# facebookresearch/gtn

Hardware: AMD Instinct MI355X
Metric: CTC forward+backward losses/sec (T=1000, C=256) (higher is better)
Workload: dtype f32; 1 GPU; BASELINE config C3: compose(ctc_target, emissions)+forwardScore CTC loss fwd+bwd, T=1000, C=256, U=100, batch=512 per GPU; global_batch=512, parallelism=dp1 (utterance sharding, all_gather of losses), rccl_ranks=0

## Files before the change

gtn_amd/csrc/band.hip:

```cpp
#include <hip/hip_runtime.h>

#include <algorithm>
#include <cstdlib>
#include <stdexcept>
#include <type_traits>

#include "kernels.h"

#ifdef GTNX_BAND_TIMING
__device__ long long g_band_timing[256];
#endif

namespace gtnx {
namespace {

constexpr float NEGF = -1.0e30f;
constexpr float DEADF = -1.0e29f;
constexpr float LOG2E = 1.44269504088896340736f;
constexpr double LN2 = 0.693147180559945309417;
constexpr int BW = 256;
constexpr int WG = 512;
constexpr int WGB = 768;
constexpr int NBE = 5;
constexpr int NBG = 7;
constexpr int NBGE = 8;
#ifndef GTNX_BWD_SPLIT
#define GTNX_BWD_SPLIT 0
#endif
#ifndef GTNX_FWD_COPY_DEPTH
// ... 323 lines not shown
    P.norm = nullptr;
    P.em_copy = nullptr;
    P.grad_em = pt.grad_em ? pt.grad_em + int64_t(b) * pt.A : nullptr;
    P.grad_fixed = pt.grad_fixed ? pt.grad_fixed + P.goff : nullptr;
  }
  return P;
}
template <int NPL, bool UNIT, bool GRADG, int K, bool VEC, bool BIG>
__global__ __launch_bounds__(WGB, BIG ? 3 : 6) void band_backward_kernel(const BandPair* __restrict__ pairs, int NSmax, BandPatch patch) {
#define GTNX_BAND_PAIR band_patched(pairs[blockIdx.x], patch)
#include "band_backward_body.inc"
#undef GTNX_BAND_PAIR
}
template <int NPL, bool UNIT, bool GRADG, int K, bool VEC, bool BIG>
__global__ __launch_bounds__(WGB, BIG ? 3 : 6) void band_backward_one_kernel(BandPair one, int NSmax) {
#define GTNX_BAND_PAIR one
#include "band_backward_body.inc"
#undef GTNX_BAND_PAIR
}


__global__ __launch_bounds__(512) void ctc_targets_kernel(const CtcTargetArgs* __restrict__ args, int blank) {
  const CtcTargetArgs a = args[blockIdx.x];
  __shared__ __attribute__((aligned(16))) int tl[256 + 4];
  __shared__ __attribute__((aligned(16))) int tk[256 + 4];
  const int N = a.N, U = (N - 1) >> 1, m = threadIdx.x;
  if (m < 260) {
    const int v = m < U ? a.labels[m] : 0x7fffffff;
    tl[m] = v;
    tk[m] = (m > 0 && m < U && v != a.labels[m - 1]) ? 1 : 0;
  }
  __syncthreads();
  if (m >= N) return;
  const bool odd = (m & 1) != 0;
  const int my = odd ? tl[(m - 1) >> 1] : blank;
  const int skip = odd ? tk[(m - 1) >> 1] : 0;
  const int mi = (m - 1) >> 1;
  const int before = odd ? mi : (m >> 1);
  int rank = 0, skips = 0;
  for (int o = 0; o < U; o += 4) {
    const gtnx_i4 l4 = *reinterpret_cast<const gtnx_i4*>(tl + o), k4 = *reinterpret_cast<const gtnx_i4*>(tk + o);
    const int lo[4] = {l4.x, l4.y, l4.z, l4.w}, ko[4] = {k4.x, k4.y, k4.z, k4.w};
#pragma unroll
    for (int k = 0; k < 4; ++k) {
      const bool front = o + k < before;
      rank += (lo[k] < my || (lo[k] == my && front)) ? 1 : 0;
      skips += front ? ko[k] : 0;
    }
  }
  rank += blank < my ? U + 1 : (blank == my ? (m + 1) >> 1 : 0);
  const int base = (m > 0 ? 2 * m - 1 : 0) + skips;
  GTNX_G BandNode* nd = const_cast<GTNX_G BandNode*>(a.nodes);
  nd[m].lab = my;
  nd[m].aid[0] = base;
  nd[m].aid[1] = m > 0 ? base + 1 : -1;
  nd[m].aid[2] = skip ? base + 2 : -1;
  a.nflags[m] = uint8_t((m == 0 ? NF_START : 0) | (m + 2 >= N ? NF_ACCEPT : 0));
  a.snode[rank] = m;
  a.slab[rank] = my;
  if (m == N - 1 && a.n_arcs) a.n_arcs[0] = base + 1 + (m > 0 ? 1 : 0) + skip;
}

__global__ __launch_bounds__(512) void band_viterbi_kernel(const BandDecode* __restrict__ pairs) {
  const BandDecode P = pairs[blockIdx.x];
  const int T = P.T, C = P.C, N = P.N, NS = P.NS;
  extern __shared__ float lds[];
  const float NINF = -__builtin_inff();
  float* a0 = lds;
  float* a1 = lds + 516;
  float* stage = lds + 1032;
  const int m = threadIdx.x;
  const GTNX_G gtnx_i4* nodes = reinterpret_cast<const GTNX_G gtnx_i4*>(P.nodes);
  int lab = 0;
  float wi[3] = {NINF, NINF, NINF};
  bool accept = false, start = false;
  if (m < N) {
    const gtnx_i4 q = nodes[m];
    lab = q.x >= 0 ? q.x : 0;
    const int a[3] = {q.y, q.z, q.w};
#pragma unroll
    for (int k = 0; k < 3; ++k)
      if (a[k] >= 0) wi[k] = P.w ? P.w[a[k]] : 0.0f;
    const uint8_t f = P.nflags[m];
// ... 565 lines not shown
```

gtn_amd/csrc/batch.cpp:

```cpp
#include "batch.h"

#include <algorithm>
#include <atomic>
#include <cstdlib>
#include <cstring>
#include <limits>
#include <unordered_map>
#include <unordered_set>

namespace gtnx {

namespace {

std::atomic<uint64_t> g_batch_seq{1};

struct CompMode {
  int old;
  CompMode() : old(compose_mode_hint(2)) {}
  ~CompMode() { compose_mode_hint(old); }
};

BatchP make_batch(Batch::Kind k, int n, bool cg) {
  auto b = std::make_shared<Batch>();
  b->kind = k;
  b->n = n;
  b->calc_grad = cg;
  return b;
}

BatchP result(Batch::Kind k, int n, std::shared_ptr<BatchOp> op) {
  bool cg = false;
  for (auto& i : op->inputs) cg |= i->calc_grad;
  BatchP r = make_batch(k, n, cg);
  op->seq = g_batch_seq.fetch_add(1);
  r->op = std::move(op);
  return r;
}

bool native(const Batch& b, Batch::Kind k) { return b.kind == k; }

void pad_fill(Batch& b, float* base, const int64_t* offs = nullptr) {
  if (b.kind != Batch::LINEAR || b.pad_floats <= 0) return;
  Runtime& rt = Runtime::get();
  const size_t n = size_t(b.n);
  const size_t rows_bytes = align_up(sizeof(int) * n, 256);
  if (!b.pad_mem) {
    std::vector<int64_t> tab(rows_bytes / 8 + n + 1);
    std::memcpy(tab.data(), b.rows.data(), sizeof(int) * n);
    int64_t* prefix = tab.data() + rows_bytes / 8;
    prefix[0] = 0;
    for (size_t i = 0; i < n; ++i) prefix[i + 1] = prefix[i] + int64_t(b.M - b.rows[i]) * b.C;
    b.pad_mem = upload_vec(tab);
  }
  PadFillArgs a{};
  a.base = base;
  a.rows = b.pad_mem->as<int>();
  a.prefix = reinterpret_cast<const int64_t*>(b.pad_mem->as<char>(rows_bytes));
  a.stride = int64_t(b.M) * b.C;
  a.n = b.n;
  a.C = b.C;
  DevMemP d_offs;
  if (offs) {
// ... 351 lines not shown
  b->lab_off.resize(size_t(n) + 1);
  b->lab_off[0] = 0;
  for (int i = 0; i < n; ++i) {
    if (lengths[i] < 0) throw_invalid("[gtnx_batch_ctc_targets] negative length");
    b->lab_off[size_t(i) + 1] = b->lab_off[size_t(i)] + lengths[i];
    b->max_nodes = std::max(b->max_nodes, 2 * lengths[i] + 1);
  }
  const size_t total = size_t(b->lab_off[size_t(n)]);
  b->labels.assign(labels, labels + total);
  int mn = blank;
  b->max_label = blank;
  for (size_t i = 0; i < total; ++i) {
    b->max_label = std::max(b->max_label, labels[i]);
    mn = std::min(mn, labels[i]);
  }
  if (mn < 0 || b->max_nodes > band_max_nodes() || n == 0) {
    std::vector<Graph> gs;
    gs.reserve(size_t(n));
    for (int i = 0; i < n; ++i)
      gs.push_back(ctc_target_graph_host(labels + b->lab_off[size_t(i)], lengths[i], blank, calc_grad));
    return batch_from_graphs(std::move(gs));
  }
  Runtime& rt = Runtime::get();
  const size_t lab_bytes = align_up(sizeof(int) * (total ? total : 1), 256);
  const size_t arg_bytes = align_up(sizeof(CtcTargetArgs) * size_t(n), 256);
  size_t bytes = lab_bytes + arg_bytes;
  b->rec_off.resize(size_t(n));
  for (int i = 0; i < n; ++i) {
    const size_t N = size_t(2 * lengths[i] + 1);
    b->rec_off[size_t(i)] = bytes;
    bytes += align_up(sizeof(BandNode) * N, 64) + align_up(N, 64) + 2 * align_up(4 * N, 64) + 64;
  }
  b->rec_mem = rt.alloc(bytes);
  PinnedMemP pin = rt.alloc_pinned(lab_bytes + arg_bytes);
  std::memcpy(pin->ptr, labels, sizeof(int) * total);
  CtcTargetArgs* args = reinterpret_cast<CtcTargetArgs*>(static_cast<char*>(pin->ptr) + lab_bytes);
  for (int i = 0; i < n; ++i) {
    const size_t N = size_t(2 * lengths[i] + 1);
    char* base = b->rec_mem->as<char>(b->rec_off[size_t(i)]);
    CtcTargetArgs& a = args[size_t(i)];
    a.labels = b->rec_mem->as<int>() + b->lab_off[size_t(i)];
    a.nodes = reinterpret_cast<BandNode*>(base);
    base += align_up(sizeof(BandNode) * N, 64);
    a.nflags = reinterpret_cast<uint8_t*>(base);
    base += align_up(N, 64);
    a.snode = reinterpret_cast<int*>(base);
    base += align_up(4 * N, 64);
    a.slab = reinterpret_cast<int*>(base);
    base += align_up(4 * N, 64);
    a.n_arcs = reinterpret_cast<int*>(base);
    a.N = int(N);
    a.pad = 0;
  }
  rt.h2d_pinned(b->rec_mem->ptr, pin->ptr, lab_bytes + arg_bytes);
  launch_ctc_targets(reinterpret_cast<const CtcTargetArgs*>(b->rec_mem->as<char>(lab_bytes)), n, blank, rt.stream());
  return b;
}


BatchP batch_asg_force_align(const int* labels, const int* lengths, int n, Graph& transitions, int n_labels) {
  if (n < 0) throw_invalid("[gtnx_batch_asg_force_align] negative batch size");
  if (transitions.num_nodes() != int64_t(n_labels) + 1 || transitions.num_arcs() != int64_t(n_labels) * (n_labels + 1))
    throw_invalid("[gtnx_batch_asg_force_align] the transitions graph must have the asgTransitions(N) layout");
  BatchP b = make_batch(Batch::CTC_TARGETS, n, transitions.calc_grad());
  b->fal = true;
  b->trans = transitions;
  b->trans_labels = n_labels;
  b->lab_off.resize(size_t(n) + 1);
  b->lab_off[0] = 0;
  int max_u = 0;
  for (int i = 0; i < n; ++i) {
    if (lengths[i] < 0) throw_invalid("[gtnx_batch_asg_force_align] negative length");
    b->lab_off[size_t(i) + 1] = b->lab_off[size_t(i)] + lengths[i];
    max_u = std::max(max_u, lengths[i]);
  }
  b->max_nodes = max_u + 1;
  const size_t total = size_t(b->lab_off[size_t(n)]);
  b->labels.assign(labels, labels + total);
// ... 520 lines not shown
      p.T = ch.rows_of(b);
      p.C = C;
      p.NS = band_row_stride(p.N, band_npl(p.N));
      p.alpha = op->arena->as<float>(ao[size_t(b)]);
      p.aoff = op->arena->as<double>(oo[size_t(b)]);
      p.score = op->arena->as<float>(4 * size_t(b));
      if (want_norm) {
        p.norm = op->arena->as<float>(o_norm + 4 * size_t(b));
        p.rowlse = op->arena->as<float>(o_lse + 4 * size_t(b) * size_t(T));
      }
      p.hot = (!fx.fal && U + 1 >= 8) ? fx.blank : -1;
      p.lgrn = band_forward_lgrn(C);
      p.bidx = b;
      p.goff = goff_run;
      goff_run += int64_t(fx.elem_size(b));
      BandPair q = p;
      if (fuse_copy) {
        q.em = static_cast<const float*>(pend->src_of(p.em));
        q.em_copy = const_cast<float*>(p.em);
      }
      tab.push_back({BandLaunchKey{C, band_npl(q.N), fx.fal ? 0 : 1, 0, band_vec_ok(q)}, q});
      abytes += 4.0 * p.T * C + 4.0 * double(p.T + 1) * p.NS + (fuse_copy ? 4.0 * T * C : 0.0);
    }
    band_launch(tab, false, "band_forward_score", abytes, fuse_copy ? nullptr : &op->fwd_table);
    if (fuse_copy) pend->done.store(true, std::memory_order_release);
    if (want_norm) {
      ch.nc_mem = op->arena;
      ch.nc_norm = op->arena->as<float>(o_norm);
      ch.nc_rowlse = op->arena->as<float>(o_lse);
    }
    DevMemP arena = op->arena;
    BatchP r = result(Batch::SCALAR, n, op);
    r->v_mem = arena;
    r->v_dev = arena->as<float>();
    return r;
  }
  if (!tropical && native(*x, Batch::LINEAR) && !x->materialised && x->nc_norm) {
    auto op = std::make_shared<BFsLinearOp>();
    op->inputs = {x};
    BatchP r = result(Batch::SCALAR, x->n, op);
    r->v_mem = x->nc_mem;
    r->v_dev = x->nc_norm;
    return r;
  }
  if (!tropical && native(*x, Batch::LINEAR) && !x->materialised && x->n > 0 && x->M > 0) {
    if (x->w_pend) x->w_pend->settle();
    auto op = std::make_shared<BFsLinearOp>();
// ... 105 lines not shown
  bool asg = x->kind == Batch::PRODUCT && x->fixed && x->chain && x->fixed->kind == Batch::CTC_TARGETS && x->fixed->fal &&
             x->chain->kind == Batch::LINEAR && x->fixed->rec_mem && x->fixed->n == n && x->chain->n == n;
  if (asg) {
    const Batch& fx = *x->fixed;
    const Batch& ch = *x->chain;
    const int vec = ch.C % 4 == 0 && (reinterpret_cast<uintptr_t>(ch.w_dev) & 15) == 0;
    asg = asg_align_ok(fx.max_nodes, ch.C, vec) && fx.trans_labels == ch.C && fx.max_label < ch.C;
  }
  if (!fast && !asg) {
    align_fallback(x, frames, labels_dev, row_stride, tokens_dev, scores_dev);
    return;
  }
  Batch& fx = *x->fixed;
  Batch& ch = *x->chain;
  const int T = ch.M, C = ch.C;
  if (row_stride < T) throw_invalid("[gtnx_batch_viterbi_align] row_stride is shorter than the chains");
  if (frames)
    for (int b = 0; b < n; ++b) {
      if (frames[b] < 0 || frames[b] > T) throw_invalid("[gtnx_batch_viterbi_align] a frame count outside 0 .. T");
      if (frames[b] > ch.rows_of(b))
        throw_invalid("[gtnx_batch_viterbi_align] a frame count beyond the rows the chain carries");
    }
  if (ch.w_pend) ch.w_pend->settle();
  if (asg) {
    const int npl = asg_align_npl(fx.max_nodes);
    const size_t plane = asg_align_plane_bytes(T, npl);
    DevMemP work = rt.alloc(plane * size_t(n));
    std::vector<AsgAlignArgs> tab(static_cast<size_t>(n));
    double abytes = 0;
    for (int b = 0; b < n; ++b) {
      AsgAlignArgs& a = tab[size_t(b)];
      a = AsgAlignArgs{};
      const int U = fx.lab_off[size_t(b) + 1] - fx.lab_off[size_t(b)];
      const size_t N = size_t(U) + 1;
      char* base = fx.rec_mem->as<char>(fx.rec_off[size_t(b)]);
      a.nodes = reinterpret_cast<BandNode*>(base);
      a.nflags = reinterpret_cast<uint8_t*>(base + align_up(sizeof(BandNode) * N, 64));
      a.w = fx.rec_mem->as<float>(fx.w_off[size_t(b)]);
      a.em = ch.w_dev + size_t(b) * size_t(T) * size_t(C);
      a.bp = work->as<unsigned>(plane * size_t(b));
      a.labels = labels_dev + int64_t(b) * row_stride;
      a.tokens = tokens_dev ? tokens_dev + int64_t(b) * row_stride : nullptr;
      a.score = scores_dev ? scores_dev + b : nullptr;
      a.N = int(N);
      a.T = frames ? frames[b] : ch.rows_of(b);
      a.T_full = T;
// ... 604 lines not shown
  const bool binary = k != SK_NEGATE;
  if (binary && a->n == b->n) {
    const bool an = a->kind == Batch::SCALAR && !a->materialised, bn = b->kind == Batch::SCALAR && !b->materialised;
    if (an && !bn && b->kind == Batch::GRAPHS) {
      if (BatchP w = scalars_from_graphs(b)) b = w;
    } else if (bn && !an && a->kind == Batch::GRAPHS) {
      if (BatchP w = scalars_from_graphs(a)) a = w;
    }
  }

  if (native(*a, Batch::SCALAR) && !a->materialised &&
      (!binary || (native(*b, Batch::SCALAR) && !b->materialised && b->n == a->n))) {
    Runtime& rt = Runtime::get();
    auto op = std::make_shared<BScalarOp>();
    op->kind = k;
    op->inputs = binary ? std::vector<BatchP>{a, b} : std::vector<BatchP>{a};
    BatchP r = result(Batch::SCALAR, a->n, op);
    if (items_dev) {
      r->v_dev = static_cast<float*>(items_dev);
    } else {
      r->v_mem = rt.alloc(sizeof(float) * size_t(a->n ? a->n : 1));
      r->v_dev = r->v_mem->as<float>();
    }
    launch_vec_axpby(r->v_dev, a->v_dev, binary ? b->v_dev : nullptr, size_t(a->n), k == SK_NEGATE ? -1.0f : 1.0f,
                     k == SK_SUBTRACT ? -1.0f : 1.0f, 0, rt.stream());
    return r;
  }
  batch_materialise(*a);
  std::vector<Graph> none;
  if (binary) batch_materialise(*b);
  BatchP r = batch_from_graphs(op_scalar(k, a->graphs, binary ? b->graphs : none));
  if (items_dev) batch_items_device(r, items_dev);
  return r;
}

void batch_backward(const BatchP& root, bool retain) {
  GTNX_HOST_T("batch.backward");
  if (root->tape_cleared)
    throw_invalid("[autograd::backward] Cannot Backward twice without retaining the graph.");
  if (root->materialised || !root->op || root->kind != Batch::SCALAR) {
    batch_materialise(*root);
    op_backward(root->graphs, nullptr, retain);
    return;
  }
  Runtime& rt = Runtime::get();
  std::vector<Batch*> order;
  std::unordered_set<Batch*> seen;
  std::vector<BatchP> hold;
  std::vector<BatchP> stack{root};
  while (!stack.empty()) {
    BatchP b = stack.back();
    stack.pop_back();
    if (!b->calc_grad || !seen.insert(b.get()).second) continue;
    hold.push_back(b);
    if (b->op) {
      order.push_back(b.get());
      for (auto& in : b->op->inputs) stack.push_back(in);
    }
  }
  std::sort(order.begin(), order.end(), [](Batch* a, Batch* b) { return a->op->seq > b->op->seq; });
  bool root_done = false;
  if (!root->g_dev) {
    alloc_grad(*root, false);
    auto* sop = dynamic_cast<BScalarOp*>(root->op.get());
    bool plain = sop != nullptr && !sop->inputs.empty() && sop->inputs.size() <= 2;
    if (plain)
      for (auto& in : sop->inputs) plain = plain && in->kind == Batch::SCALAR && !in->materialised && in->n == root->n;
    if (plain && sop->inputs.size() == 2 && sop->inputs[0].get() == sop->inputs[1].get()) plain = false;
    if (plain) {
      float* g[2] = {nullptr, nullptr};
      float sc[2] = {0.0f, 0.0f};
      int acc[2] = {0, 0};
      for (size_t i = 0; i < sop->inputs.size(); ++i) {
        Batch& in = *sop->inputs[i];
        if (!in.calc_grad) continue;
        sc[i] = (sop->kind == SK_NEGATE || (sop->kind == SK_SUBTRACT && i == 1)) ? -1.0f : 1.0f;
        acc[i] = in.g_dev != nullptr;
        if (!in.g_dev) alloc_grad(in, false);
        g[i] = in.g_dev;
      }
      launch_scalar_seed(root->g_dev, g[0], sc[0], acc[0], g[1], sc[1], acc[1], size_t(root->n), rt.stream());
      root_done = true;
    } else {
      launch_fill_f32(root->g_dev, 1.0f, size_t(root->n), rt.stream());
    }
  } else {
    DevMemP ones = rt.alloc(sizeof(float) * size_t(root->n ? root->n : 1));
    launch_fill_f32(ones->as<float>(), 1.0f, size_t(root->n), rt.stream());
    launch_vec_axpby(root->g_dev, ones->as<float>(), nullptr, size_t(root->n), 1.0f, 0.0f, 1, rt.stream());
  }
  std::vector<Batch*> from_graphs;
  BackwardPlan plan;
  t_plan = &plan;
  struct RetainScope {
    bool prev;
    explicit RetainScope(bool r) : prev(t_batch_retain) { t_batch_retain = r; }
    ~RetainScope() { t_batch_retain = prev; }
  } retain_scope(retain);
  try {
    for (Batch* b : order) {
      if (!b->g_dev) continue;
      if (root_done && b == root.get()) continue;
      if (auto* f = dynamic_cast<BFromGraphsOp*>(b->op.get())) {
        f->retain = retain;
        from_graphs.push_back(b);
        continue;
// ... 114 lines not shown
```

gtn_amd/csrc/batch.h:

```cpp
#pragma once

#include <memory>
#include <vector>

#include "ops.h"

namespace gtnx {

struct Batch;
using BatchP = std::shared_ptr<Batch>;

struct BatchOp {
  uint64_t seq = 0;
  std::vector<BatchP> inputs;
  virtual void backward(Batch& out) = 0;
  virtual ~BatchOp() {}
};

struct Batch {
  enum Kind { GRAPHS, CTC_TARGETS, LINEAR, PRODUCT, SCALAR };
  Kind kind = GRAPHS;
  int n = 0;
  bool calc_grad = false;

  bool materialised = false;
  std::vector<Graph> graphs;
  bool leaf = false;
  struct Origin {
    std::shared_ptr<void> home;
    size_t begin, end;
  };
  std::vector<Origin> origins;
  void (*give_back)(const std::shared_ptr<void>& home, std::vector<Graph>* part) = nullptr;
  std::vector<float> host_vals;
  bool host_vals_valid = false;
  PinnedMemP host_pin;
  void* host_ev = nullptr;

  std::vector<int> labels, lab_off;
  int blank = 0;
  int max_label = -1, max_nodes = 0;
  DevMemP rec_mem;
  std::vector<size_t> rec_off;
  bool fal = false;
  Graph trans;
  int trans_labels = 0;
  std::vector<size_t> w_off, map_off;
  int M = 0, C = 0;
  DevMemP w_mem;
  float* w_dev = nullptr;
  std::shared_ptr<PendingCopy> w_pend;
  DevMemP nc_mem;
  float* nc_norm = nullptr;
  float* nc_rowlse = nullptr;
  std::vector<int> rows;
  int64_t pad_floats = 0;
  DevMemP pad_mem;
  int rows_of(int b) const { return rows.empty() ? M : rows[size_t(b)]; }
  BatchP fixed, chain;
  bool chain_first = false, intersect = false;
  bool wide = false;
  bool full = false;
  DevMemP v_mem;
  float* v_dev = nullptr;

  std::shared_ptr<BatchOp> op;
  bool tape_cleared = false;
  DevMemP g_mem;
  float* g_dev = nullptr;
  std::vector<int64_t> g_off;
  DevMemP dest_mem;
  float* dest = nullptr;

  int64_t elem_size(int b) const;
  ~Batch();
};

BatchP batch_from_graphs(std::vector<Graph> gs);
BatchP batch_ctc_targets(const int* labels, const int* lengths, int n, int blank, bool calc_grad);
BatchP batch_asg_force_align(const int* labels, const int* lengths, int n, Graph& transitions, int n_labels);
BatchP batch_linear(int n, int M, int C, bool calc_grad, const void* dev, bool borrow, const int* rows = nullptr);
BatchP batch_compose(const BatchP& a, const BatchP& b, bool intersect);
BatchP batch_shortest_distance(const BatchP& x, bool tropical);
void batch_full_connect_stats(int64_t* fast, int64_t* fallback);
BatchP batch_viterbi_path(const BatchP& x);
void batch_viterbi_align(const BatchP& x, const int* frames, int* labels_dev, int64_t row_stride, int* tokens_dev,
                         float* scores_dev);
// ... 35 lines not shown
```

gtn_amd/csrc/kernels.h:

```cpp
#pragma once

#include <hip/hip_runtime.h>

#include <cstdint>

#include <atomic>
#include <cstdint>
struct gtnx_first_on_device {
  std::atomic<uint64_t>& done;
  uint64_t bit;
  bool first;
  explicit gtnx_first_on_device(std::atomic<uint64_t>& d) : done(d) {
    int dev = 0;
    (void)hipGetDevice(&dev);
    bit = uint64_t(1) << (dev & 63);
    first = !(done.load(std::memory_order_acquire) & bit);
  }
  gtnx_first_on_device(const gtnx_first_on_device&) = delete;
  ~gtnx_first_on_device() {
    if (first) done.fetch_or(bit, std::memory_order_acq_rel);
  }
  explicit operator bool() const { return first; }
};

// ... 449 lines not shown
  GTNX_G int* stamp;
  GTNX_G int* queue;
  GTNX_G int* arc_cnt;
  const GTNX_G int* arc_off;
  RationalOut out;
};
void launch_remove_keep(const DGraph& g, int ilabel, int olabel, int* keep, hipStream_t st);
void launch_remove_roots(const int* keep, const int* new_id, int N, int* roots, hipStream_t st);
void launch_remove_walk(const RemoveArgs& a, bool emit, hipStream_t st);
size_t scan_temp_bytes(int n);
void launch_exclusive_scan(const int* in, int* out, int n, void* temp, size_t temp_bytes, hipStream_t st);
void launch_rational_load(const void* rows, const float* w, const uint8_t* flags, const RationalOut& out, void* temp,
                          hipStream_t st);
struct CtcTargetArgs {
  const GTNX_G int* labels;
  GTNX_G BandNode* nodes;
  GTNX_G uint8_t* nflags;
  GTNX_G int* snode;
  GTNX_G int* slab;
  GTNX_G int* n_arcs;
  int N, pad;
};
void launch_ctc_targets(const CtcTargetArgs* d_args, int n, int blank, hipStream_t st);
struct AsgFalArgs {
  const GTNX_G int* labels;
  const GTNX_G float* trans_w;
  GTNX_G BandNode* nodes;
  GTNX_G uint8_t* nflags;
  GTNX_G int* snode;
  GTNX_G int* slab;
  GTNX_G float* w;
  GTNX_G int* arc_map;
  int U, pad;
};
void launch_asg_fal_targets(const AsgFalArgs* d_args, int n, int n_labels, hipStream_t st);
void launch_asg_fal_scatter(const float* g, const int* maps, const int64_t* tab , int n_seq, int64_t longest,
                            float* trans_grad, hipStream_t st);
int band_max_nodes();
int band_max_labels();
int band_min_labels();
int band_npl(int max_nodes);
int band_row_stride(int N, int npl);
int band_forward_lgrn(int C);
bool band_one_ok(int npl, int C, int max_NS, bool vec, bool backward);
void launch_band_forward(const BandPair* d_pairs, int n, int npl, int C, int max_NS, bool unit, bool vec, hipStream_t st,
                         const BandPair* one = nullptr);
// ... 5 lines not shown
void launch_lazy_dense_fixed_grad(const LazyGroup& g, hipStream_t st);
size_t maxplus_w_floats(const LazyGroup& g);
void launch_maxplus_prep(const LazyGroup& g, hipStream_t st);
void launch_maxplus_step(const LazyGroup& g, int t, hipStream_t st);
void launch_maxplus_path(const LazyGroup& g, int* path_arc, int* path_il, int* path_ol, float* path_w, int* path_len,
                         hipStream_t st);
void launch_asg_decode(const LazyGroup& g, const int* d_frames, int* labels, int64_t row_stride, float* scores,
                       int* collapsed, int* lengths, hipStream_t st);
void launch_lazy_mfma_prep(const LazyGroup& g, hipStream_t st);
void launch_lazy_mfma_init(const LazyGroup& g, int which, hipStream_t st);
void launch_lazy_mfma_step(const LazyGroup& g, int t, int backward, hipStream_t st);
size_t lazy_mfma_chain_sync_ints(const LazyGroup& g);
bool launch_lazy_mfma_chain(const LazyGroup& g, int backward, int* zeroed_sync, int cus, hipStream_t st);
void launch_lazy_mfma_keys(float* keys, int64_t n, hipStream_t st);
void launch_lazy_mfma_rowmax(const LazyGroup& g, int which, hipStream_t st);
void launch_lazy_mfma_score(const LazyGroup& g, hipStream_t st);
size_t lazy_mfma_fixed_grad_scratch_bytes(const LazyGroup& g);
void launch_lazy_mfma_fixed_grad(const LazyGroup& g, void* pair_consts , hipStream_t st, void* partials = nullptr,
                                 size_t partials_bytes = 0);

void launch_fill_i32(int* p, int v, size_t n, hipStream_t st);
void launch_fill_f32(float* p, float v, size_t n, hipStream_t st);
void launch_scalar_seed(float* root, float* g0, float s0, int acc0, float* g1, float s1, int acc1, size_t n, hipStream_t st);
struct ScalarArgs {
  const GTNX_G float* a;
  const GTNX_G float* b;
  GTNX_G float* out;
  GTNX_G float* mirror;
};
void launch_scalar_combine(const ScalarArgs* d_args, int n, float sa, float sb, hipStream_t st);
void launch_copy_small(void* dst, const void* src, size_t bytes, hipStream_t st);
void launch_scalar_combine_one(const ScalarArgs& a, float sa, float sb, hipStream_t st);
struct ScalarFanArgs {
  const GTNX_G float* d;
  GTNX_G float* seed;
  GTNX_G float* o0;
  GTNX_G float* o1;
};
void launch_scalar_fan(const ScalarFanArgs* d_args, int n, float s0, float s1, hipStream_t st);
void launch_scalar_fan_one(const ScalarFanArgs& a, float s0, float s1, hipStream_t st);
struct AxpyArgs {
  GTNX_G float* dst;
  const GTNX_G float* src;
  int64_t n;
  float scale;
};
// ... 104 lines not shown
```

gtn_amd/csrc/ops.h:

```cpp
#pragma once

#include <cstring>
#include <tuple>
#include <vector>

#include "graph.h"

namespace gtnx {

struct Member {
  int idx;
  Graph out;
};

struct OpRecord {
  uint64_t seq = 0;
  virtual void backward(std::vector<Member>& members) = 0;
  virtual bool joins_chain_plan() const { return false; }
  virtual ~OpRecord() {}
};

struct GradSink {
  struct Item {
    Graph g;
    DevMemP owner;
    float* ptr;
  };
  std::vector<Item> items;
  void add(const Graph& g, const DevMemP& owner, float* ptr) {
    if (g.calc_grad()) items.push_back({g, owner, ptr});
  }
  void flush();
};

struct BandLaunchKey {
  int C, npl, unit, gradg, vec;
  bool operator<(const BandLaunchKey& o) const {
    return std::tie(C, npl, unit, gradg, vec) < std::tie(o.C, o.npl, o.unit, o.gradg, o.vec);
  }
  bool operator==(const BandLaunchKey& o) const { return !(*this < o) && !(o < *this); }
};
int band_vec_ok(const BandPair& p);
void band_launch(std::vector<std::pair<BandLaunchKey, BandPair>>& tab, bool backward, const char* prof_name = nullptr,
                 double prof_bytes = 0.0, DevMemP* table_out = nullptr);
void band_launch_patched(const DevMemP& table, int n, const BandLaunchKey& key, int max_ns, const BandPatch& patch,
                         const char* prof_name, double prof_bytes);

enum ScalarKind { SK_NEGATE = 0, SK_ADD = 1, SK_SUBTRACT = 2 };

std::vector<Graph> op_scalar(ScalarKind k, std::vector<Graph>& a, std::vector<Graph>& b);
std::vector<Graph> op_shortest_distance(std::vector<Graph>& gs, bool tropical);
std::vector<Graph> op_viterbi_path(std::vector<Graph>& gs);
std::vector<Graph> op_compose(std::vector<Graph>& a, std::vector<Graph>& b, bool intersect);
bool lazy_decode_ok(Graph& fixed, int M, int C);
void lazy_viterbi_decode(std::vector<Graph>& chains, Graph& fixed, const std::vector<int>& frames, int* labels_dev,
                         int64_t row_stride, float* scores_dev, int* collapsed_dev, int* lengths_dev);
enum RationalKind { RAT_CLONE = 0, RAT_CONCAT = 1, RAT_CLOSURE = 2, RAT_UNION = 3 };
Graph op_rational(int kind, std::vector<Graph>& inputs, int projection);
Graph op_remove(Graph& g, int ilabel, int olabel);
Graph op_load_buffer(const void* data, size_t bytes);
void op_backward(std::vector<Graph>& roots, Graph* grad, bool retain, bool seed = true);
void backward_validate(Graph& root);
int compose_mode_hint(int mode);
void realize(Graph& g);

Graph make_scalar_graph(float v, bool calc_grad);
Graph make_linear_graph(int M, int N, bool calc_grad);
// ... 41 lines not shown
```

gtn_amd/csrc/ops_band.cpp:

```cpp
#include "ops_internal.h"

#include <memory>

namespace gtnx {

int band_vec_ok(const BandPair& p) { return p.C % 4 == 0 && (reinterpret_cast<uintptr_t>(p.em) & 15) == 0; }
void band_launch_patched(const DevMemP& table, int n, const BandLaunchKey& k, int max_ns, const BandPatch& patch,
                         const char* prof_name, double prof_bytes) {
  Runtime& rt = Runtime::get();
  std::unique_ptr<Runtime::Scope> prof(prof_name ? new Runtime::Scope(&rt, prof_name, prof_bytes) : nullptr);
  launch_band_backward(table->as<BandPair>(), n, k.npl, k.C, max_ns, k.unit != 0, k.gradg != 0, k.vec != 0, rt.stream(), nullptr,
                       &patch);
}
void band_launch(std::vector<std::pair<BandLaunchKey, BandPair>>& tab, bool backward, const char* prof_name, double prof_bytes,
                 DevMemP* table_out) {
  Runtime& rt = Runtime::get();
  if (table_out) table_out->reset();
  if (tab.empty()) return;
  bool one_key = true;
  for (size_t i = 1; i < tab.size() && one_key; ++i) one_key = tab[i].first == tab[0].first;
  if (!one_key) std::stable_sort(tab.begin(), tab.end(), [](const auto& x, const auto& y) { return x.first < y.first; });
  if (tab.size() == 1) {
    const BandLaunchKey& k = tab[0].first;
    const BandPair& p = tab[0].second;
    if (band_one_ok(k.npl, k.C, p.NS, k.vec != 0, backward)) {
      std::unique_ptr<Runtime::Scope> prof(prof_name ? new Runtime::Scope(&rt, prof_name, prof_bytes) : nullptr);
      if (backward) launch_band_backward(nullptr, 1, k.npl, k.C, p.NS, k.unit != 0, k.gradg != 0, true, rt.stream(), &p);
      else launch_band_forward(nullptr, 1, k.npl, k.C, p.NS, k.unit != 0, true, rt.stream(), &p);
      return;
    }
  }
  std::vector<BandPair> flat;
  flat.reserve(tab.size());
  for (auto& e : tab) flat.push_back(e.second);
  DevMemP d = upload_vec(flat);
// ... 692 lines not shown
```

gtn_amd/csrc/runtime.cpp:

```cpp
#include "runtime.h"

#include "kernels.h"

#include <malloc.h>

#include <atomic>
#include <condition_variable>
#include <cstring>
#include <deque>
#include <thread>

namespace gtnx {

namespace {
constexpr int kMaxDevices = 64;
std::atomic<Runtime*> g_rts[kMaxDevices];
std::atomic<bool> g_any_rt{false};
std::mutex g_rt_mu;
std::atomic<int> g_default_device{-1};
thread_local int t_device = -1;

int hip_device_now() {
  int d = -1;
  if (hipGetDevice(&d) != hipSuccess) {
// ... 562 lines not shown
    (void)hipGetLastError();
    return false;
  }
  return a.type == hipMemoryTypeHost || (a.type == hipMemoryTypeDevice && a.device == dev);
}
}
bool ptr_local_to(const void* p, int dev) { return local_to(p, dev); }
void Runtime::d2d(void* dst, const void* src, size_t bytes) {
  if (!bytes) return;
  if (bytes <= (size_t(1) << 20) && local_to(src, device_) && local_to(dst, device_)) {
    launch_copy_small(dst, src, bytes, stream_);
    return;
  }
  HIP_CHECK(hipMemcpyAsync(dst, src, bytes, hipMemcpyDeviceToDevice, stream_));
}
void Runtime::d2h_pinned_async(void* pinned_dst, const void* src, size_t bytes) {
  if (!bytes) return;
  if (bytes <= (size_t(1) << 20) && local_to(src, device_)) {
    launch_copy_small(pinned_dst, src, bytes, stream_);
    return;
  }
  HIP_CHECK(hipMemcpyAsync(pinned_dst, src, bytes, hipMemcpyDeviceToHost, stream_));
}
void Runtime::h2d_pinned(void* dst, const void* pinned_src, size_t bytes) {
  if (!bytes) return;
  static const size_t lim = [] {
    const char* e = std::getenv("GTNX_H2D_KERNEL_BYTES");
    return e ? size_t(std::atol(e)) : size_t(1) << 20;
  }();
  if (bytes <= lim && local_to(dst, device_)) {
    launch_copy_small(dst, pinned_src, bytes, stream_);
    return;
  }
  HIP_CHECK(hipMemcpyAsync(dst, pinned_src, bytes, hipMemcpyHostToDevice, stream_));
}

Runtime::MirrorSlot Runtime::mirror_slot() {
  {
    std::lock_guard<std::mutex> lk(mu_);
    if (!mirror_ring_) {
      OnDevice here(device_);
      void* p = nullptr;
      HIP_CHECK(hipHostMalloc(&p, sizeof(float) * kMirrorSlots, hipHostMallocDefault));
      mirror_gen_ = new std::atomic<uint64_t>[kMirrorSlots];
      for (size_t i = 0; i < kMirrorSlots; ++i) mirror_gen_[i].store(0);
      mirror_ring_ = static_cast<float*>(p);
    }
  }
  const uint64_t g = mirror_next_.fetch_add(1) + 1;
  const size_t i = size_t(g % kMirrorSlots);
  mirror_gen_[i].store(g);
  return {mirror_ring_ + i, g};
// ... 126 lines not shown
```

gtn_amd/csrc/runtime.h:

```cpp
#pragma once

#include <atomic>
#include <functional>
#include <map>
#include <memory>
#include <mutex>
#include <string>
#include <vector>

#include "common.h"

namespace gtnx {

class Runtime;

struct DevMem {
  void* ptr = nullptr;
  size_t bytes = 0;
  bool borrowed = false;
  Runtime* owner = nullptr;
  std::shared_ptr<void> keep;
  ~DevMem();
  template <class T>
  T* as(size_t byte_off = 0) const { return reinterpret_cast<T*>(static_cast<char*>(ptr) + byte_off); }
// ... 46 lines not shown
    bool dead = false;
  };
  using InboxP = std::shared_ptr<Inbox>;
  static InboxP home();
  static void send(const InboxP& to, void* p, void (*del)(void*));
  static void drain_all_inboxes();
  static void defer_delete(void* p, void (*del)(void*), size_t weight = 1);
  static void drain_deferred();
  static bool drain_some(size_t max_items);
  static size_t deferred_count();
  void drain_until(void* hip_event);
  void drain_while_busy();
  void sync_while_draining();

  struct SideJob;
  using SideJobP = std::shared_ptr<SideJob>;
  SideJobP side_launch(std::function<void(hipStream_t)> fn);
  void side_join(const SideJobP& job);

  void h2d(void* dst, const void* src, size_t bytes);
  void d2h_sync(void* dst, const void* src, size_t bytes);
  void d2d(void* dst, const void* src, size_t bytes);
  void h2d_pinned(void* dst, const void* pinned_src, size_t bytes);
  void d2h_pinned_async(void* pinned_dst, const void* src, size_t bytes);

  struct MirrorSlot {
    float* ptr = nullptr;
    uint64_t gen = 0;
  };
  static constexpr size_t kMirrorSlots = 1024;
  MirrorSlot mirror_slot();
  bool mirror_read(const MirrorSlot& m, float* out);

  void prof_enable(bool on);
  void prof_add_bytes(const std::string& name, double bytes);
  void prof_reset();
  bool prof_on() const { return prof_on_; }
  struct Scope {
    Runtime* rt;
    int idx;
    Scope(Runtime* r, const char* name, double bytes);
    ~Scope();
  };
  ProfEntry prof_get(const std::string& name);
  std::string prof_names();
  int cu_count() const { return cu_count_; }
// ... 56 lines not shown
```

Before: 1.036 million losses/s.

## Fuse CTC target staging, pair-table upload and loss seeding into fewer launches

The CTC target builder now reads labels and args directly from pinned host staging inside a single head kernel. That kernel also copies the forward band pair table, so the separate H2D copy and table upload launches are folded into it and deferred until the forward score launch. For the subtract loss, a fused seed kernel computes the difference and writes the root and input gradient seeds at once, and backward adopts these instead of launching a fill or seed kernel. This cuts kernel launch and host overhead per step but adds state (head_pin, seed_mem) and an env switch, and the kernels now read host-pinned memory over the bus.

```diff
diff --git a/gtn_amd/csrc/band.hip b/gtn_amd/csrc/band.hip
--- a/gtn_amd/csrc/band.hip
+++ b/gtn_amd/csrc/band.hip
@@ -5,6 +5,7 @@
 #include <stdexcept>
 #include <type_traits>
 
+#include "ctc_targets_build.h"
 #include "kernels.h"
 
 #ifdef GTNX_BAND_TIMING
@@ -374,43 +375,7 @@
 
 __global__ __launch_bounds__(512) void ctc_targets_kernel(const CtcTargetArgs* __restrict__ args, int blank) {
   const CtcTargetArgs a = args[blockIdx.x];
-  __shared__ __attribute__((aligned(16))) int tl[256 + 4];
-  __shared__ __attribute__((aligned(16))) int tk[256 + 4];
-  const int N = a.N, U = (N - 1) >> 1, m = threadIdx.x;
-  if (m < 260) {
-    const int v = m < U ? a.labels[m] : 0x7fffffff;
-    tl[m] = v;
-    tk[m] = (m > 0 && m < U && v != a.labels[m - 1]) ? 1 : 0;
-  }
-  __syncthreads();
-  if (m >= N) return;
-  const bool odd = (m & 1) != 0;
-  const int my = odd ? tl[(m - 1) >> 1] : blank;
-  const int skip = odd ? tk[(m - 1) >> 1] : 0;
-  const int mi = (m - 1) >> 1;
-  const int before = odd ? mi : (m >> 1);
-  int rank = 0, skips = 0;
-  for (int o = 0; o < U; o += 4) {
-    const gtnx_i4 l4 = *reinterpret_cast<const gtnx_i4*>(tl + o), k4 = *reinterpret_cast<const gtnx_i4*>(tk + o);
-    const int lo[4] = {l4.x, l4.y, l4.z, l4.w}, ko[4] = {k4.x, k4.y, k4.z, k4.w};
-#pragma unroll
-    for (int k = 0; k < 4; ++k) {
-      const bool front = o + k < before;
-      rank += (lo[k] < my || (lo[k] == my && front)) ? 1 : 0;
-      skips += front ? ko[k] : 0;
-    }
-  }
-  rank += blank < my ? U + 1 : (blank == my ? (m + 1) >> 1 : 0);
-  const int base = (m > 0 ? 2 * m - 1 : 0) + skips;
-  GTNX_G BandNode* nd = const_cast<GTNX_G BandNode*>(a.nodes);
-  nd[m].lab = my;
-  nd[m].aid[0] = base;
-  nd[m].aid[1] = m > 0 ? base + 1 : -1;
-  nd[m].aid[2] = skip ? base + 2 : -1;
-  a.nflags[m] = uint8_t((m == 0 ? NF_START : 0) | (m + 2 >= N ? NF_ACCEPT : 0));
-  a.snode[rank] = m;
-  a.slab[rank] = my;
-  if (m == N - 1 && a.n_arcs) a.n_arcs[0] = base + 1 + (m > 0 ? 1 : 0) + skip;
+  ctc_targets_build<false>(a, a.labels, blank);
 }
 
 __global__ __launch_bounds__(512) void band_viterbi_kernel(const BandDecode* __restrict__ pairs) {
diff --git a/gtn_amd/csrc/batch.cpp b/gtn_amd/csrc/batch.cpp
--- a/gtn_amd/csrc/batch.cpp
+++ b/gtn_amd/csrc/batch.cpp
@@ -1,4 +1,5 @@
 #include "batch.h"
+#include "ctc_head.h"
 
 #include <algorithm>
 #include <atomic>
@@ -38,6 +39,36 @@
 }
 
 bool native(const Batch& b, Batch::Kind k) { return b.kind == k; }
+
+bool step_fused() {
+  static const bool on = [] {
+    const char* e = std::getenv("GTNX_STEP_LAUNCHES");
+    return !(e && std::atoi(e) == 7);
+  }();
+  return on;
+}
+
+void launch_head(Batch& fx, const BandPair* pairs, DevMemP* table) {
+  Runtime& rt = Runtime::get();
+  CtcHeadArgs h{};
+  h.stage = fx.head_pin->ptr;
+  h.dev = fx.rec_mem->ptr;
+  h.arg_off = fx.head_arg_off;
+  h.n = fx.n;
+  h.blank = fx.blank;
+  if (pairs) {
+    h.pair_bytes = ctc_head_put_pairs(fx.head_pair_off, fx.head_pin->ptr, pairs, fx.n);
+    DevMemP d = rt.alloc(h.pair_bytes);
+    h.pair_src = fx.head_pin->as<char>(fx.head_pair_off);
+    h.pair_dst = d->ptr;
+    *table = std::move(d);
+  }
+  launch_ctc_head(h, rt.stream());
+  fx.head_pin.reset();
+}
+void settle_head(Batch& fx) {
+  if (fx.head_pin) launch_head(fx, nullptr, nullptr);
+}
 
 void pad_fill(Batch& b, float* base, const int64_t* offs = nullptr) {
   if (b.kind != Batch::LINEAR || b.pad_floats <= 0) return;
@@ -435,38 +466,20 @@
     return batch_from_graphs(std::move(gs));
   }
   Runtime& rt = Runtime::get();
-  const size_t lab_bytes = align_up(sizeof(int) * (total ? total : 1), 256);
-  const size_t arg_bytes = align_up(sizeof(CtcTargetArgs) * size_t(n), 256);
-  size_t bytes = lab_bytes + arg_bytes;
-  b->rec_off.resize(size_t(n));
-  for (int i = 0; i < n; ++i) {
-    const size_t N = size_t(2 * lengths[i] + 1);
-    b->rec_off[size_t(i)] = bytes;
-    bytes += align_up(sizeof(BandNode) * N, 64) + align_up(N, 64) + 2 * align_up(4 * N, 64) + 64;
-  }
-  b->rec_mem = rt.alloc(bytes);
-  PinnedMemP pin = rt.alloc_pinned(lab_bytes + arg_bytes);
-  std::memcpy(pin->ptr, labels, sizeof(int) * total);
-  CtcTargetArgs* args = reinterpret_cast<CtcTargetArgs*>(static_cast<char*>(pin->ptr) + lab_bytes);
-  for (int i = 0; i < n; ++i) {
-    const size_t N = size_t(2 * lengths[i] + 1);
-    char* base = b->rec_mem->as<char>(b->rec_off[size_t(i)]);
-    CtcTargetArgs& a = args[size_t(i)];
-    a.labels = b->rec_mem->as<int>() + b->lab_off[size_t(i)];
-    a.nodes = reinterpret_cast<BandNode*>(base);
-    base += align_up(sizeof(BandNode) * N, 64);
-    a.nflags = reinterpret_cast<uint8_t*>(base);
-    base += align_up(N, 64);
-    a.snode = reinterpret_cast<int*>(base);
-    base += align_up(4 * N, 64);
-    a.slab = reinterpret_cast<int*>(base);
-    base += align_up(4 * N, 64);
-    a.n_arcs = reinterpret_cast<int*>(base);
-    a.N = int(N);
-    a.pad = 0;
-  }
-  rt.h2d_pinned(b->rec_mem->ptr, pin->ptr, lab_bytes + arg_bytes);
-  launch_ctc_targets(reinterpret_cast<const CtcTargetArgs*>(b->rec_mem->as<char>(lab_bytes)), n, blank, rt.stream());
+  const CtcHeadLayout lay = ctc_head_layout(lengths, n, total);
+  b->rec_off = lay.rec_off;
+  b->rec_mem = rt.alloc(lay.dev_bytes);
+  const bool head = step_fused() && n > 1 && lay.stage_bytes(true) <= Runtime::h2d_kernel_limit();
+  PinnedMemP pin = rt.alloc_pinned(lay.stage_bytes(head));
+  ctc_head_fill(lay, pin->ptr, b->rec_mem->ptr, labels, b->lab_off.data(), lengths, n);
+  if (head) {
+    b->head_pin = std::move(pin);
+    b->head_arg_off = lay.lab_bytes;
+    b->head_pair_off = lay.pair_off();
+    return b;
+  }
+  rt.h2d_pinned(b->rec_mem->ptr, pin->ptr, lay.stage_bytes(false));
+  launch_ctc_targets(reinterpret_cast<const CtcTargetArgs*>(b->rec_mem->as<char>(lay.lab_bytes)), n, blank, rt.stream());
   return b;
 }
 
@@ -1033,7 +1046,24 @@
       tab.push_back({BandLaunchKey{C, band_npl(q.N), fx.fal ? 0 : 1, 0, band_vec_ok(q)}, q});
       abytes += 4.0 * p.T * C + 4.0 * double(p.T + 1) * p.NS + (fuse_copy ? 4.0 * T * C : 0.0);
     }
-    band_launch(tab, false, "band_forward_score", abytes, fuse_copy ? nullptr : &op->fwd_table);
+    bool one_group = n > 1;
+    int max_ns = 0;
+    for (auto& e : tab) {
+      one_group = one_group && e.first == tab[0].first;
+      max_ns = std::max(max_ns, e.second.NS);
+    }
+    if (fx.head_pin && one_group) {
+      std::vector<BandPair> flat;
+      flat.reserve(tab.size());
+      for (auto& e : tab) flat.push_back(e.second);
+      DevMemP table;
+      launch_head(fx, flat.data(), &table);
+      if (!fuse_copy) op->fwd_table = table;
+      band_launch_forward_table(table, n, tab[0].first, max_ns, "band_forward_score", abytes);
+    } else {
+      settle_head(fx);
+      band_launch(tab, false, "band_forward_score", abytes, fuse_copy ? nullptr : &op->fwd_table);
+    }
     if (fuse_copy) pend->done.store(true, std::memory_order_release);
     if (want_norm) {
       ch.nc_mem = op->arena;
@@ -1185,6 +1215,7 @@
         throw_invalid("[gtnx_batch_viterbi_align] a frame count beyond the rows the chain carries");
     }
   if (ch.w_pend) ch.w_pend->settle();
+  settle_head(fx);
   if (asg) {
     const int npl = asg_align_npl(fx.max_nodes);
     const size_t plane = asg_align_plane_bytes(T, npl);
@@ -1835,6 +1866,15 @@
       r->v_mem = rt.alloc(sizeof(float) * size_t(a->n ? a->n : 1));
       r->v_dev = r->v_mem->as<float>();
     }
+    if (k == SK_SUBTRACT && step_fused() && r->calc_grad && a->n > 0 && a.get() != b.get()) {
+      const size_t n = size_t(a->n), part = align_up(sizeof(float) * n, 256) / sizeof(float);
+      r->seed_mem = rt.alloc(sizeof(float) * part * 3);
+      float* sd = r->seed_mem->as<float>();
+      for (int i = 0; i < 3; ++i) r->seed_off[i] = part * size_t(i);
+      launch_loss_seed(r->v_dev, a->v_dev, b->v_dev, 1.0f, -1.0f, sd, a->calc_grad ? sd + part : nullptr, 1.0f,
+                       b->calc_grad ? sd + 2 * part : nullptr, -1.0f, n, rt.stream());
+      return r;
+    }
     launch_vec_axpby(r->v_dev, a->v_dev, binary ? b->v_dev : nullptr, size_t(a->n), k == SK_NEGATE ? -1.0f : 1.0f,
                      k == SK_SUBTRACT ? -1.0f : 1.0f, 0, rt.stream());
     return r;
@@ -1874,13 +1914,30 @@
   std::sort(order.begin(), order.end(), [](Batch* a, Batch* b) { return a->op->seq > b->op->seq; });
   bool root_done = false;
   if (!root->g_dev) {
-    alloc_grad(*root, false);
     auto* sop = dynamic_cast<BScalarOp*>(root->op.get());
     bool plain = sop != nullptr && !sop->inputs.empty() && sop->inputs.size() <= 2;
     if (plain)
       for (auto& in : sop->inputs) plain = plain && in->kind == Batch::SCALAR && !in->materialised && in->n == root->n;
     if (plain && sop->inputs.size() == 2 && sop->inputs[0].get() == sop->inputs[1].get()) plain = false;
-    if (plain) {
+    bool seeded = plain && root->seed_mem && !root->dest && sop->kind == SK_SUBTRACT && sop->inputs.size() == 2;
+    if (seeded)
+      for (auto& in : sop->inputs) seeded = seeded && !(in->calc_grad && (in->g_dev || in->dest));
+    if (seeded) {
+      auto adopt = [&](Batch& x, size_t off) {
+        x.g_off.resize(size_t(x.n) + 1);
+        for (int i = 0; i <= x.n; ++i) x.g_off[size_t(i)] = i;
+        x.g_mem = root->seed_mem;
+        x.g_dev = root->seed_mem->as<float>() + off;
+      };
+      for (size_t i = 0; i < 2; ++i)
+        if (sop->inputs[i]->calc_grad) adopt(*sop->inputs[i], root->seed_off[i + 1]);
+      adopt(*root, root->seed_off[0]);
+      root->seed_mem.reset();
+      root_done = true;
+    } else {
+      alloc_grad(*root, false);
+    }
+    if (!seeded && plain) {
       float* g[2] = {nullptr, nullptr};
       float sc[2] = {0.0f, 0.0f};
       int acc[2] = {0, 0};
@@ -1894,7 +1951,7 @@
       }
       launch_scalar_seed(root->g_dev, g[0], sc[0], acc[0], g[1], sc[1], acc[1], size_t(root->n), rt.stream());
       root_done = true;
-    } else {
+    } else if (!seeded) {
       launch_fill_f32(root->g_dev, 1.0f, size_t(root->n), rt.stream());
     }
   } else {
diff --git a/gtn_amd/csrc/batch.h b/gtn_amd/csrc/batch.h
--- a/gtn_amd/csrc/batch.h
+++ b/gtn_amd/csrc/batch.h
@@ -42,6 +42,8 @@
   int max_label = -1, max_nodes = 0;
   DevMemP rec_mem;
   std::vector<size_t> rec_off;
+  PinnedMemP head_pin;
+  size_t head_arg_off = 0, head_pair_off = 0;
   bool fal = false;
   Graph trans;
   int trans_labels = 0;
@@ -63,6 +65,8 @@
   bool full = false;
   DevMemP v_mem;
   float* v_dev = nullptr;
+  DevMemP seed_mem;
+  size_t seed_off[3] = {0, 0, 0};
 
   std::shared_ptr<BatchOp> op;
   bool tape_cleared = false;
diff --git a/gtn_amd/csrc/ctc_head.h b/gtn_amd/csrc/ctc_head.h
--- /dev/null
+++ b/gtn_amd/csrc/ctc_head.h
@@ -0,0 +1,75 @@
+#pragma once
+
+#include <cstddef>
+#include <cstring>
+#include <vector>
+
+#include "common.h"
+#include "kernels.h"
+
+namespace gtnx {
+
+struct CtcHeadLayout {
+  size_t lab_bytes = 0;
+  size_t arg_bytes = 0;
+  size_t pair_bytes = 0;
+  size_t dev_bytes = 0;
+  std::vector<size_t> rec_off;
+  size_t stage_bytes(bool with_pairs) const { return lab_bytes + arg_bytes + (with_pairs ? pair_bytes : 0); }
+  size_t pair_off() const { return lab_bytes + arg_bytes; }
+};
+
+inline size_t ctc_head_record_bytes(size_t N) {
+  return align_up(sizeof(BandNode) * N, 64) + align_up(N, 64) + 2 * align_up(4 * N, 64) + 64;
+}
+
+inline CtcHeadLayout ctc_head_layout(const int* lengths, int n, size_t total_labels) {
+  CtcHeadLayout L;
+  L.lab_bytes = align_up(sizeof(int) * (total_labels ? total_labels : 1), 256);
+  L.arg_bytes = align_up(sizeof(CtcTargetArgs) * size_t(n), 256);
+  L.pair_bytes = align_up(sizeof(BandPair) * size_t(n), 256);
+  size_t bytes = L.lab_bytes + L.arg_bytes;
+  L.rec_off.resize(size_t(n));
+  for (int i = 0; i < n; ++i) {
+    L.rec_off[size_t(i)] = bytes;
+    bytes += ctc_head_record_bytes(size_t(2 * lengths[i] + 1));
+  }
+  L.dev_bytes = bytes;
+  return L;
+}
+
+inline void ctc_head_fill(const CtcHeadLayout& L, void* stage, void* dev, const int* labels, const int* lab_off,
+                          const int* lengths, int n) {
+  char* s = static_cast<char*>(stage);
+  char* d = static_cast<char*>(dev);
+  const size_t total = size_t(lab_off[n]);
+  if (total) std::memcpy(s, labels, sizeof(int) * total);
+  CtcTargetArgs* args = reinterpret_cast<CtcTargetArgs*>(s + L.lab_bytes);
+  for (int i = 0; i < n; ++i) {
+    const size_t N = size_t(2 * lengths[i] + 1);
+    char* base = d + L.rec_off[size_t(i)];
+    CtcTargetArgs& a = args[size_t(i)];
+    a.labels = reinterpret_cast<int*>(d) + lab_off[i];
+    a.nodes = reinterpret_cast<BandNode*>(base);
+    base += align_up(sizeof(BandNode) * N, 64);
+    a.nflags = reinterpret_cast<uint8_t*>(base);
+    base += align_up(N, 64);
+    a.snode = reinterpret_cast<int*>(base);
+    base += align_up(4 * N, 64);
+    a.slab = reinterpret_cast<int*>(base);
+    base += align_up(4 * N, 64);
+    a.n_arcs = reinterpret_cast<int*>(base);
+    a.N = int(N);
+    a.pad = 0;
+  }
+}
+
+inline size_t ctc_head_put_pairs(size_t pair_off, void* stage, const BandPair* pairs, int n) {
+  const size_t bytes = sizeof(BandPair) * size_t(n), padded = align_up(bytes, 16);
+  char* dst = static_cast<char*>(stage) + pair_off;
+  std::memcpy(dst, pairs, bytes);
+  std::memset(dst + bytes, 0, padded - bytes);
+  return padded;
+}
+
+}
diff --git a/gtn_amd/csrc/ctc_head.hip b/gtn_amd/csrc/ctc_head.hip
--- /dev/null
+++ b/gtn_amd/csrc/ctc_head.hip
@@ -0,0 +1,62 @@
+#include <hip/hip_runtime.h>
+
+#include <cstdint>
+
+#include "ctc_targets_build.h"
+#include "kernels.h"
+
+namespace gtnx {
+namespace {
+
+constexpr int kHeadBlock = 512;
+
+__global__ __launch_bounds__(kHeadBlock) void ctc_head_kernel(CtcHeadArgs h) {
+  if (int(blockIdx.x) >= h.n) {
+    const size_t n16 = h.pair_bytes >> 4, stride = size_t(gridDim.x - h.n) * kHeadBlock;
+    const uint4* src = static_cast<const uint4*>(h.pair_src);
+    uint4* dst = static_cast<uint4*>(h.pair_dst);
+    for (size_t i = size_t(blockIdx.x - h.n) * kHeadBlock + threadIdx.x; i < n16; i += stride) dst[i] = src[i];
+    return;
+  }
+  const CtcTargetArgs* staged = reinterpret_cast<const CtcTargetArgs*>(static_cast<const char*>(h.stage) + h.arg_off);
+  const CtcTargetArgs a = staged[blockIdx.x];
+  if (threadIdx.x == 0) reinterpret_cast<CtcTargetArgs*>(static_cast<char*>(h.dev) + h.arg_off)[blockIdx.x] = a;
+  const size_t lab_off = reinterpret_cast<uintptr_t>(a.labels) - reinterpret_cast<uintptr_t>(h.dev);
+  ctc_targets_build<true>(a, reinterpret_cast<const int*>(static_cast<const char*>(h.stage) + lab_off), h.blank);
+}
+
+__global__ void loss_seed_kernel(float* out, const float* a, const float* b, float sa, float sb, float* root, float* g0,
+                                 float s0, float* g1, float s1, size_t n) {
+  for (size_t i = blockIdx.x * size_t(blockDim.x) + threadIdx.x; i < n; i += size_t(gridDim.x) * blockDim.x) {
+    float v = sa * a[i];
+    v += sb * b[i];
+    out[i] = v;
+    root[i] = 1.0f;
+    if (g0) g0[i] = s0;
+    if (g1) g1[i] = s1;
+  }
+}
+
+}
+
+int ctc_head_pair_groups(size_t pair_bytes) {
+  const size_t per = size_t(kHeadBlock) * 16;
+  const size_t g = (pair_bytes + per - 1) / per;
+  return int(g > 256 ? 256 : g);
+}
+
+void launch_ctc_head(const CtcHeadArgs& h, hipStream_t st) {
+  if (h.n <= 0) return;
+  const int extra = h.pair_bytes ? ctc_head_pair_groups(h.pair_bytes) : 0;
+  hipLaunchKernelGGL(ctc_head_kernel, dim3(unsigned(h.n + extra)), dim3(kHeadBlock), 0, st, h);
+}
+
+void launch_loss_seed(float* out, const float* a, const float* b, float sa, float sb, float* root, float* g0, float s0,
+                      float* g1, float s1, size_t n, hipStream_t st) {
+  if (!n) return;
+  const size_t g = (n + 255) / 256;
+  hipLaunchKernelGGL(loss_seed_kernel, dim3(unsigned(g > 4096 ? 4096 : g)), dim3(256), 0, st, out, a, b, sa, sb, root, g0,
+                     s0, g1, s1, n);
+}
+
+}
diff --git a/gtn_amd/csrc/ctc_targets_build.h b/gtn_amd/csrc/ctc_targets_build.h
--- /dev/null
+++ b/gtn_amd/csrc/ctc_targets_build.h
@@ -0,0 +1,55 @@
+#pragma once
+
+#include <hip/hip_runtime.h>
+
+#include "kernels.h"
+
+namespace gtnx {
+
+template <bool STAGED, class LabelPtr>
+__device__ __forceinline__ void ctc_targets_build(const CtcTargetArgs& a, LabelPtr labels, int blank) {
+  __shared__ __attribute__((aligned(16))) int tl[256 + 4];
+  __shared__ __attribute__((aligned(16))) int tk[256 + 4];
+  const int N = a.N, U = (N - 1) >> 1, m = threadIdx.x;
+  if (m < 260) {
+    const int v = m < U ? labels[m] : 0x7fffffff;
+    tl[m] = v;
+    if (!STAGED) tk[m] = (m > 0 && m < U && v != labels[m - 1]) ? 1 : 0;
+    if (STAGED && m < U) const_cast<GTNX_G int*>(a.labels)[m] = v;
+  }
+  __syncthreads();
+  if (STAGED) {
+    if (m < 260) tk[m] = (m > 0 && m < U && tl[m] != tl[m - 1]) ? 1 : 0;
+    __syncthreads();
+  }
+  if (m >= N) return;
+  const bool odd = (m & 1) != 0;
+  const int my = odd ? tl[(m - 1) >> 1] : blank;
+  const int skip = odd ? tk[(m - 1) >> 1] : 0;
+  const int mi = (m - 1) >> 1;
+  const int before = odd ? mi : (m >> 1);
+  int rank = 0, skips = 0;
+  for (int o = 0; o < U; o += 4) {
+    const gtnx_i4 l4 = *reinterpret_cast<const gtnx_i4*>(tl + o), k4 = *reinterpret_cast<const gtnx_i4*>(tk + o);
+    const int lo[4] = {l4.x, l4.y, l4.z, l4.w}, ko[4] = {k4.x, k4.y, k4.z, k4.w};
+#pragma unroll
+    for (int k = 0; k < 4; ++k) {
+      const bool front = o + k < before;
+      rank += (lo[k] < my || (lo[k] == my && front)) ? 1 : 0;
+      skips += front ? ko[k] : 0;
+    }
+  }
+  rank += blank < my ? U + 1 : (blank == my ? (m + 1) >> 1 : 0);
+  const int base = (m > 0 ? 2 * m - 1 : 0) + skips;
+  GTNX_G BandNode* nd = const_cast<GTNX_G BandNode*>(a.nodes);
+  nd[m].lab = my;
+  nd[m].aid[0] = base;
+  nd[m].aid[1] = m > 0 ? base + 1 : -1;
+  nd[m].aid[2] = skip ? base + 2 : -1;
+  a.nflags[m] = uint8_t((m == 0 ? NF_START : 0) | (m + 2 >= N ? NF_ACCEPT : 0));
+  a.snode[rank] = m;
+  a.slab[rank] = my;
+  if (m == N - 1 && a.n_arcs) a.n_arcs[0] = base + 1 + (m > 0 ? 1 : 0) + skip;
+}
+
+}
diff --git a/gtn_amd/csrc/kernels.h b/gtn_amd/csrc/kernels.h
--- a/gtn_amd/csrc/kernels.h
+++ b/gtn_amd/csrc/kernels.h
@@ -495,6 +495,17 @@
   int N, pad;
 };
 void launch_ctc_targets(const CtcTargetArgs* d_args, int n, int blank, hipStream_t st);
+struct CtcHeadArgs {
+  const void* stage;
+  void* dev;
+  size_t arg_off;
+  const void* pair_src;
+  void* pair_dst;
+  size_t pair_bytes;
+  int n, blank;
+};
+void launch_ctc_head(const CtcHeadArgs& a, hipStream_t st);
+int ctc_head_pair_groups(size_t pair_bytes);
 struct AsgFalArgs {
   const GTNX_G int* labels;
   const GTNX_G float* trans_w;
@@ -546,6 +557,8 @@
 void launch_fill_i32(int* p, int v, size_t n, hipStream_t st);
 void launch_fill_f32(float* p, float v, size_t n, hipStream_t st);
 void launch_scalar_seed(float* root, float* g0, float s0, int acc0, float* g1, float s1, int acc1, size_t n, hipStream_t st);
+void launch_loss_seed(float* out, const float* a, const float* b, float sa, float sb, float* root, float* g0, float s0,
+                      float* g1, float s1, size_t n, hipStream_t st);
 struct ScalarArgs {
   const GTNX_G float* a;
   const GTNX_G float* b;
diff --git a/gtn_amd/csrc/ops.h b/gtn_amd/csrc/ops.h
--- a/gtn_amd/csrc/ops.h
+++ b/gtn_amd/csrc/ops.h
@@ -43,6 +43,8 @@
 int band_vec_ok(const BandPair& p);
 void band_launch(std::vector<std::pair<BandLaunchKey, BandPair>>& tab, bool backward, const char* prof_name = nullptr,
                  double prof_bytes = 0.0, DevMemP* table_out = nullptr);
+void band_launch_forward_table(const DevMemP& table, int n, const BandLaunchKey& key, int max_ns, const char* prof_name,
+                               double prof_bytes);
 void band_launch_patched(const DevMemP& table, int n, const BandLaunchKey& key, int max_ns, const BandPatch& patch,
                          const char* prof_name, double prof_bytes);
 
diff --git a/gtn_amd/csrc/ops_band.cpp b/gtn_amd/csrc/ops_band.cpp
--- a/gtn_amd/csrc/ops_band.cpp
+++ b/gtn_amd/csrc/ops_band.cpp
@@ -11,6 +11,12 @@
   std::unique_ptr<Runtime::Scope> prof(prof_name ? new Runtime::Scope(&rt, prof_name, prof_bytes) : nullptr);
   launch_band_backward(table->as<BandPair>(), n, k.npl, k.C, max_ns, k.unit != 0, k.gradg != 0, k.vec != 0, rt.stream(), nullptr,
                        &patch);
+}
+void band_launch_forward_table(const DevMemP& table, int n, const BandLaunchKey& k, int max_ns, const char* prof_name,
+                               double prof_bytes) {
+  Runtime& rt = Runtime::get();
+  std::unique_ptr<Runtime::Scope> prof(prof_name ? new Runtime::Scope(&rt, prof_name, prof_bytes) : nullptr);
+  launch_band_forward(table->as<BandPair>(), n, k.npl, k.C, max_ns, k.unit != 0, k.vec != 0, rt.stream());
 }
 void band_launch(std::vector<std::pair<BandLaunchKey, BandPair>>& tab, bool backward, const char* prof_name, double prof_bytes,
                  DevMemP* table_out) {
diff --git a/gtn_amd/csrc/runtime.cpp b/gtn_amd/csrc/runtime.cpp
--- a/gtn_amd/csrc/runtime.cpp
+++ b/gtn_amd/csrc/runtime.cpp
@@ -608,12 +608,16 @@
   }
   HIP_CHECK(hipMemcpyAsync(pinned_dst, src, bytes, hipMemcpyDeviceToHost, stream_));
 }
-void Runtime::h2d_pinned(void* dst, const void* pinned_src, size_t bytes) {
-  if (!bytes) return;
+size_t Runtime::h2d_kernel_limit() {
   static const size_t lim = [] {
     const char* e = std::getenv("GTNX_H2D_KERNEL_BYTES");
     return e ? size_t(std::atol(e)) : size_t(1) << 20;
   }();
+  return lim;
+}
+void Runtime::h2d_pinned(void* dst, const void* pinned_src, size_t bytes) {
+  if (!bytes) return;
+  const size_t lim = h2d_kernel_limit();
   if (bytes <= lim && local_to(dst, device_)) {
     launch_copy_small(dst, pinned_src, bytes, stream_);
     return;
diff --git a/gtn_amd/csrc/runtime.h b/gtn_amd/csrc/runtime.h
--- a/gtn_amd/csrc/runtime.h
+++ b/gtn_amd/csrc/runtime.h
@@ -92,6 +92,7 @@
   void d2h_sync(void* dst, const void* src, size_t bytes);
   void d2d(void* dst, const void* src, size_t bytes);
   void h2d_pinned(void* dst, const void* pinned_src, size_t bytes);
+  static size_t h2d_kernel_limit();
   void d2h_pinned_async(void* pinned_dst, const void* src, size_t bytes);
 
   struct MirrorSlot {
```

New measurement: 996,100 losses/s. 3.9% lower.
